# c-zhou/oatk

Measured on AMD Instinct MI355X. Metric: HiFi Gbases/s through syncasm (syncmer+syncerr) at k=1001 s=31, higher is better.
Workload: dtype u64

## Files before the change

oatk_amd/csrc/scan_syncmer_fast.hpp:

```cpp
#pragma once
#include <type_traits>
#include "common.hpp"
#include "scan_syncmer.hpp"
#include "scan_hpc.hpp"

namespace oatk {

constexpr int SYF_C = 8;
constexpr int SYF_T = SYN_NT * SYF_C;
constexpr int SYF_BLK = 64;
constexpr int SYF_LIST = 128;

static inline int syncmer_fast_ring(int K, int S)
{
    const int w = K - S;
    if (w / SYF_C - 1 < SYF_BLK || w / SYF_C - 1 >= 2 * SYF_BLK) return 0;
    if (K + SYF_T + SYF_C + 64 <= 4096) return 4096;
    return 0;
}

#define OATK_DPP_ROW_SHL(n) (0x100 + (n))
#define OATK_DPP_ROW_SHR(n) (0x110 + (n))
#define OATK_DPP_ROW_BCAST15 0x142
#define OATK_DPP_ROW_BCAST31 0x143

template <int CTRL, int ROW_MASK = 0xf>
__device__ __forceinline__ uint32_t dpp_u32(uint32_t old, uint32_t src)
{
    return (uint32_t) __builtin_amdgcn_update_dpp((int) old, (int) src, CTRL, ROW_MASK, 0xf, false);
}

__device__ __forceinline__ uint32_t wave_prefix_min_u32(uint32_t v)
{
    uint32_t p = v, t;
    t = dpp_u32<OATK_DPP_ROW_SHR(1)>(0xFFFFFFFFu, p); p = t < p? t : p;
    t = dpp_u32<OATK_DPP_ROW_SHR(2)>(0xFFFFFFFFu, p); p = t < p? t : p;
    t = dpp_u32<OATK_DPP_ROW_SHR(4)>(0xFFFFFFFFu, p); p = t < p? t : p;
    t = dpp_u32<OATK_DPP_ROW_SHR(8)>(0xFFFFFFFFu, p); p = t < p? t : p;
    t = dpp_u32<OATK_DPP_ROW_BCAST15, 0xa>(0xFFFFFFFFu, p); p = t < p? t : p;
    t = dpp_u32<OATK_DPP_ROW_BCAST31, 0xc>(0xFFFFFFFFu, p); p = t < p? t : p;
    return p;
}
__device__ __forceinline__ uint32_t wave_suffix_min_mirrored_u32(uint32_t v, uint32_t lane)
{
    return wave_prefix_min_u32((uint32_t) __builtin_amdgcn_ds_bpermute((int) ((63u - lane) << 2), (int) v));
}

#define OATK_SYF_PADW(R) ((R) / 8)
#ifndef OATK_SYF_EXP
#define OATK_SYF_EXP 0
#endif
#ifndef OATK_SYF_WAVES
#define OATK_SYF_WAVES 6
#endif
template <int R, bool S31, int NT, int SH>
__global__ __launch_bounds__(NT, OATK_SYF_WAVES) void syncmer_fast_kernel(SynArgs a)
{
    constexpr int C = SYF_C, T = NT * SYF_C, NCH = R / C, NWAVE = NT / OATK_WAVE;
    static_assert((R & (R - 1)) == 0, "power-of-two ring: index arithmetic is one AND (a 3200-slot ring raised occupancy from 3 to 4\n"
                  "workgroups per CU but its modulo arithmetic cost more issue slots than the occupancy returned)");

    __shared__ uint32_t m_top[R + OATK_SYF_PADW(R)];
    __shared__ uint64_t c_min[NCH];
    __shared__ uint32_t s_tie[2];
    __shared__ uint32_t pre32[NCH], suf32[NCH];
    __shared__ uint32_t w_cnt[2][NWAVE];
    __shared__ uint32_t sl_e[SYF_LIST];
    __shared__ uint32_t s_gb;

    const uint32_t r = blockIdx.x, tid = threadIdx.x, lane = tid & 63, wid = tid >> 6;
    if (a.n_nn[r] != 0) return;

    const int K = a.K, S = S31? 31 : a.S, w = K - S;
    const uint32_t hl = a.hoco_l[r];
    if (hl < (uint32_t) K) { if (tid == 0) a.n_scm[r] = 0; return; }
    const uint64_t sid = a.sid0 + r;
    const uint64_t mask = (1ULL << (2 * S)) - 1;
    const uint32_t *ghs = (const uint32_t *) (a.hoco_s + (a.off[r] >> 2));
    const int D = w / C - 1;

    auto rpos = [](int32_t i) -> uint32_t { return (uint32_t) i & (uint32_t) (R - 1); };
    auto mi = [&](int32_t i) -> uint32_t { const uint32_t p = rpos(i); return p + ((p >> 5) << 2); };
    auto rch = [](int32_t c) -> uint32_t { return (uint32_t) c & (uint32_t) (NCH - 1); };
    for (uint32_t i = tid; i < R + OATK_SYF_PADW(R); i += NT) m_top[i] = 0xFFFFFFFFu;
    for (uint32_t i = tid; i < NCH; i += NT) pre32[i] = suf32[i] = 0xFFFFFFFFu, c_min[i] = UINT64_MAX;
    if (tid < 2) s_tie[tid] = 0;
    __syncthreads();

    struct __attribute__((packed, aligned(4))) Words3 { uint32_t a, b, c; };
    const uint32_t bsel = (tid & 1u)? 0x06070001u : 0x04050607u;
    const uint32_t last_w = (hl - 1u) >> 4;
    uint32_t rw0, rw1, rw2;
    {
        const int32_t wi0 = ((int32_t) (tid * C) - 32) >> 4;
        rw0 = ghs[wi0 < 0? 0 : wi0], rw1 = ghs[wi0 + 1 < 0? 0 : wi0 + 1], rw2 = ghs[wi0 + 2];
    }

    uint32_t ord0 = 0, par = 0;
    uint32_t sl_n = 0;
    const uint32_t lcap = hl < (1u << 30)? (uint32_t) a.list_cap : 0u;
    const int HW = (w & (C - 1)) + C;

    auto get64g = [&](int32_t t) -> uint64_t {
        const uint32_t wi = (uint32_t) t >> 4, sh = ((uint32_t) t & 15u) * 2u;
        const uint64_t hi = (uint64_t) __builtin_bswap32(ghs[wi]) << 32 | __builtin_bswap32(ghs[wi + 1]);
        const uint32_t w2 = __builtin_bswap32(ghs[wi + 2]);
        return sh? (hi << sh) | ((uint64_t) w2 >> (32u - sh)) : hi;
    };
    auto hash_at = [&](int32_t q) -> uint64_t {
        if (q + 1 < S || (uint32_t) q >= hl) return UINT64_MAX;
        const uint64_t X = get64g(q - S + 1) & (~0ULL << (64 - 2 * S));
        const uint64_t fw = X >> (64 - 2 * S), rv = revcomp32(X) & mask;
        return S31? hash64_s31(fw < rv? fw : rv) : (fw != rv? hash64(fw < rv? fw : rv, mask) : UINT64_MAX);
    };
    auto write_record = [&](int32_t E, uint32_t kind, uint32_t loc, uint32_t ordn) __attribute__((always_inline)) {
        const int32_t e = kind == 2u? E - w : E, j = E - K + 1;
        const uint64_t X = get64g(e - S + 1) & (~0ULL << (64 - 2 * S));
        const uint64_t fw = X >> (64 - 2 * S), rv = revcomp32(X) & mask;
        uint64_t code = fw < rv? fw << 1 : rv << 1 | 1ULL;
        const uint32_t rev = (uint32_t) (code & 1ULL);
        if (kind == 1u) code ^= 1ULL;
        if (loc < a.region_cap) {
            const size_t slot = (size_t) (blockIdx.x & (OATK_REC_SHARDS - 1)) * a.region_cap + loc;
            a.rec_lo[slot] = sid << 32 | (uint64_t) ordn << 1 | rev;
            a.rec_smer[slot] = code;
            a.rec_mpos[slot] = (uint32_t) j << 1 | rev;
        }
    };
    auto emit_list = [&]() __attribute__((always_inline)) {
        if (sl_n) {
            if (tid == 0) s_gb = atomicAdd(&a.shard_cnt[blockIdx.x & (OATK_REC_SHARDS - 1)], sl_n);
            __syncthreads();
            const uint32_t gb = s_gb;
            for (uint32_t i = tid; i < sl_n; i += NT) write_record((int32_t) (sl_e[i] & 0x3FFFFFFFu), sl_e[i] >> 30, gb + i, ord0 + i);
            __syncthreads();
        }
        ord0 += sl_n, sl_n = 0;
    };

    uint32_t pend_kinds = 0, pend_rank = 0, pend_wtot = 0, pend_par = 0, pend_any = 0;
    int32_t pend_i0 = 0;
    auto flush = [&]() __attribute__((always_inline)) {
        if (!pend_any) return;
        uint32_t before = 0, tot = 0;
#pragma unroll
        for (int ww = 0; ww < NWAVE; ++ww) { const uint32_t c = w_cnt[pend_par][ww]; tot += c; before += ww < (int) wid? c : 0u; }
        pend_any = 0;
        if (tot == 0) return;
        if (sl_n + tot > lcap) emit_list();
        const bool direct = tot > lcap;
        if (direct) {
            if (tid == 0) s_gb = atomicAdd(&a.shard_cnt[blockIdx.x & (OATK_REC_SHARDS - 1)], tot);
            __syncthreads();
            uint32_t rank = before + pend_rank, kk = pend_kinds;
            while (kk) {
                const int o = __builtin_ctz(kk) >> 1;
                const uint32_t kind = (pend_kinds >> (2 * o)) & 3u;
                kk &= ~(3u << (2 * o));
                write_record(pend_i0 + o, kind, s_gb + rank, ord0 + rank);
                ++rank;
            }
            __syncthreads();
        } else if (pend_wtot) {
            uint32_t idx = sl_n + before + pend_rank, kk = pend_kinds;
            while (kk) {
                const int o = __builtin_ctz(kk) >> 1;
                sl_e[idx] = (uint32_t) (pend_i0 + o) | ((pend_kinds >> (2 * o)) & 3u) << 30;
                kk &= ~(3u << (2 * o));
                ++idx;
            }
        }
        ord0 += direct? tot : 0u;
        sl_n += direct? 0u : tot;
    };

    static_assert(2 * T == R, "the address toggling below needs tile = half the ring");
    struct RangeAddr { uint32_t lo, hi, mid; bool whole; };
    auto range_addr = [&](int32_t lo, int32_t hi) -> RangeAddr {
        return RangeAddr{rch(lo) * 4u, rch(hi) * 4u, rch(((lo >> 6) + 1) * 64 + 63) * 4u, (hi >> 6) - (lo >> 6) == 2};
    };
    const int32_t ch_0 = (int32_t) tid, ca0_0 = ((int32_t) (tid * C) - w) >> 3;
    RangeAddr rB = range_addr(ch_0 - D, ch_0 - 1), rF0 = range_addr(ca0_0 + 1, ca0_0 + D), rF1 = range_addr(ca0_0 + 2, ca0_0 + 1 + D);
    uint32_t o_cs = rch(ch_0) * 4u;
    uint32_t m_own = mi((int32_t) (tid * C)), m_fa = mi(ca0_0 * C), m_fb = mi((ca0_0 + 1) * C);
    const uint32_t m_own_sum = m_own + mi((int32_t) (tid * C) + T), m_fa_sum = m_fa + mi(ca0_0 * C + T), m_fb_sum = m_fb + mi((ca0_0 + 1) * C + T);
    auto next_tile_addr = [&]() __attribute__((always_inline)) {
        constexpr uint32_t FLIP = (uint32_t) (NCH / 2) * 4u;
        o_cs ^= FLIP;
        rB.lo ^= FLIP, rB.hi ^= FLIP, rB.mid ^= FLIP, rF0.lo ^= FLIP, rF0.hi ^= FLIP, rF0.mid ^= FLIP, rF1.lo ^= FLIP, rF1.hi ^= FLIP, rF1.mid ^= FLIP;
        m_own = m_own_sum - m_own, m_fa = m_fa_sum - m_fa, m_fb = m_fb_sum - m_fb;
    };
    auto ld32 = [](const uint32_t *base, uint32_t byte_off) -> uint32_t { return *(const uint32_t *) ((const char *) base + byte_off); };

    bool rep_mode = false, rep_next = false;
    int32_t rep_start = 0x7FFFFFFF;
    uint32_t quiet = 0, tpar = 0;
    const int32_t wave_first = __builtin_amdgcn_readfirstlane((int) (wid * OATK_WAVE * C));
    uint32_t I0 = 0;
    for (; I0 + (uint32_t) wave_first < hl; I0 += T, next_tile_addr(), tpar ^= 1u) {
        if (rep_next != rep_mode) { rep_mode = rep_next; rep_start = rep_mode? (int32_t) (I0 / C) : 0x7FFFFFFF; }
        const int32_t i0 = (int32_t) (I0 + tid * C);
        const int32_t wb = (int32_t) I0 + wave_first;
        const int32_t ch = i0 / C;
        uint32_t y[C];
        uint32_t cmin_keep;
        {
            const uint32_t a_hi = __builtin_amdgcn_perm(rw0, rw1, bsel), a_lo = __builtin_amdgcn_perm(rw1, rw2, bsel);
            const uint32_t vbh = __builtin_amdgcn_perm(rw2, 0u, bsel);
            const uint64_t vb = (uint64_t) vbh << 32;
            {
                const uint32_t wn = ((I0 + T + tid * C) - 32u) >> 4;
                const Words3 nx = *(const Words3 *) (ghs + (wn < last_w? wn : last_w));
                rw0 = nx.a, rw1 = nx.b, rw2 = nx.c;
            }
            uint64_t cm = UINT64_MAX;
            uint32_t cmin = 0xFFFFFFFFu;
            const bool inside = wb + 1 >= S && (uint32_t) (wb + OATK_WAVE * C) <= hl;
            if (S31 || inside) {
                if (S31) {
                    auto rc16 = [](uint32_t x) -> uint32_t {
                        const uint32_t r = __builtin_bitreverse32(x);
                        return ~(((r >> 1) & 0x55555555u) | ((r & 0x55555555u) << 1));
                    };
                    const uint32_t r0 = rc16(a_hi), r1 = rc16(a_lo), r2 = rc16(vbh);
                    auto hash_chunk = [&](auto keep, auto ends) __attribute__((always_inline)) {
#pragma unroll
                        for (int b = 0; b < C; ++b) {
                            uint64_t fw = (uint64_t) __builtin_amdgcn_alignbit(a_hi, a_lo, 28 - 2 * b) << 32 | __builtin_amdgcn_alignbit(a_lo, vbh, 28 - 2 * b);
                            uint64_t rv = (uint64_t) __builtin_amdgcn_alignbit(r2, r1, 2 + 2 * b) << 32 | __builtin_amdgcn_alignbit(r1, r0, 2 + 2 * b);
                            asm("" : "+v"(fw), "+v"(rv));
                            const uint64_t cn = fw < rv? fw : rv;
                            uint64_t mv4 = hash64_s31_left(cn);
                            y[b] = (uint32_t) (mv4 >> 34);
                            if (decltype(ends)::value) {
                                const bool ok = i0 + b + 1 >= S && (uint32_t) (i0 + b) < hl;
                                y[b] = ok? y[b] : 0xFFFFFFFFu;
                                if (decltype(keep)::value) mv4 = ok? mv4 : UINT64_MAX;
                            }
                            cmin = y[b] < cmin? y[b] : cmin;
                            if (decltype(keep)::value) cm = mv4 < cm? mv4 : cm;
                        }
                        if (decltype(keep)::value) cm = decltype(ends)::value && cm == UINT64_MAX? cm : cm >> 2;
                    };
                    if (inside) {
                        if (__builtin_amdgcn_readfirstlane((int) rep_mode)) hash_chunk(std::true_type(), std::false_type()); else hash_chunk(std::false_type(), std::false_type());
                    } else {
                        if (__builtin_amdgcn_readfirstlane((int) rep_mode)) hash_chunk(std::true_type(), std::true_type()); else hash_chunk(std::false_type(), std::true_type());
                    }
                } else {
                    const uint64_t X = ((uint64_t) a_hi << 32 | a_lo) << (2 * (32 - S));
                    uint64_t fw = X >> (64 - 2 * S), rv = revcomp32(X) & mask;
#pragma unroll
                    for (int b = 0; b < C; ++b) {
                        const uint64_t c = (vbh >> (30 - 2 * b)) & 3u;
                        fw = (fw << 2 | c) & mask;
                        rv = rv >> 2 | (3ULL ^ c) << (2 * S - 2);
                        const uint64_t mv = fw != rv? hash64(fw < rv? fw : rv, mask) : UINT64_MAX;
                        y[b] = (uint32_t) (mv >> 32);
                        cmin = y[b] < cmin? y[b] : cmin;
                        cm = mv < cm? mv : cm;
                    }
                }
            } else {
                const uint64_t X = ((uint64_t) a_hi << 32 | a_lo) << (2 * (32 - S));
                uint64_t fw = X >> (64 - 2 * S), rv = revcomp32(X) & mask;
#pragma unroll
                for (int b = 0; b < C; ++b) {
                    const int32_t i = i0 + b;
                    const uint64_t c = (vb >> (62 - 2 * b)) & 3ULL;
                    fw = (fw << 2 | c) & mask;
                    rv = rv >> 2 | (3ULL ^ c) << (2 * S - 2);
                    uint64_t mv = UINT64_MAX;
                    if (i + 1 >= S && (uint32_t) i < hl && fw != rv) mv = S31? hash64_s31(fw < rv? fw : rv) : hash64(fw < rv? fw : rv, mask);
                    y[b] = (uint32_t) (mv >> 32);
                    cmin = y[b] < cmin? y[b] : cmin;
                    if (rep_mode) cm = mv < cm? mv : cm;
                }
            }
            cmin_keep = cmin;
            uint32_t pre, suf;
#ifdef OATK_SCAN_SHFL
            pre = suf = cmin;
            for (int d = 1; d < OATK_WAVE; d <<= 1) {
                uint32_t up = __shfl_up(pre, d), dn = __shfl_down(suf, d);
                if ((int) lane >= d) pre = up < pre? up : pre;
                if ((int) lane + d < OATK_WAVE) suf = dn < suf? dn : suf;
            }
#else
            pre = wave_prefix_min_u32(cmin);
            suf = wave_suffix_min_mirrored_u32(cmin, lane);
#endif
            __syncthreads();
            static_assert(C == 8, "two 16-byte stores per lane");
            *(uint4 *) (m_top + m_own) = make_uint4(y[0], y[1], y[2], y[3]);
            *(uint4 *) (m_top + m_own + 4) = make_uint4(y[4], y[5], y[6], y[7]);
            if (rep_mode) *(uint64_t *) ((char *) c_min + 2u * o_cs) = cm;
            {
                const uint32_t seen = s_tie[tpar ^ 1u];
                quiet = seen? 0u : quiet + 1u;
                rep_next = seen != 0u || (rep_mode && quiet < 2u);
            }
            *(uint32_t *) ((char *) pre32 + o_cs) = pre;
#ifdef OATK_SCAN_SHFL
            *(uint32_t *) ((char *) suf32 + o_cs) = suf;
#else
            *(uint32_t *) ((char *) suf32 + (o_cs ^ 252u)) = suf;
#endif
        }
        __syncthreads();
        if (tid == 0) s_tie[tpar ^ 1u] = 0;
        flush();

        static_assert(SH >= 0 && SH < C, "the window's alignment against the chunks is a template argument");
        constexpr int RR = (C - SH) & (C - 1);
        uint32_t backF_keep = 0, fwd0_keep = 0, fwd1_keep = 0;
        uint32_t kinds = 0;
        uint32_t tiemask = 0;
        if (!(wb + OATK_WAVE * C < K)) {
            auto range_min = [&](const RangeAddr &ra) -> uint32_t {
                const uint32_t a0 = ld32(suf32, ra.lo), a1 = ld32(pre32, ra.hi);
                const uint32_t mid = ld32(pre32, ra.mid);
                const uint32_t a2 = ra.whole? mid : 0xFFFFFFFFu;
                const uint32_t v = a0 < a1? a0 : a1;
                return a2 < v? a2 : v;
            };
            const uint32_t backF = range_min(rB);
            const uint32_t fwd0 = range_min(rF0);
            const uint32_t fwd1 = range_min(rF1);
            backF_keep = backF, fwd0_keep = fwd0, fwd1_keep = fwd1;
            constexpr int BD = RR? RR : C;
            uint32_t W[2 * C];
            {
                const uint4 a0 = *(const uint4 *) (m_top + m_fa), a1 = *(const uint4 *) (m_top + m_fa + 4);
                const uint4 b0 = *(const uint4 *) (m_top + m_fb), b1 = *(const uint4 *) (m_top + m_fb + 4);
                const uint32_t all[2 * C] = {a0.x, a0.y, a0.z, a0.w, a1.x, a1.y, a1.z, a1.w, b0.x, b0.y, b0.z, b0.w, b1.x, b1.y, b1.z, b1.w};
#pragma unroll
                for (int j = 0; j < 2 * C - SH; ++j) W[j] = all[SH + j];
            }
            uint32_t cprev = 0xFFFFFFFFu;
            if (RR > 0) {
                const uint32_t nb = dpp_u32<0x138>(0xFFFFFFFFu, cmin_keep);
                const uint32_t lb = ld32(suf32, (o_cs - 4u) & (uint32_t) (NCH * 4 - 1));
                cprev = lane == 0? lb : nb;
            }
            const bool edge = !(wb + 1 >= K && (uint32_t) (wb + OATK_WAVE * C) <= hl);
            auto decide = [&](auto at_edge) __attribute__((always_inline)) {
#pragma unroll
                for (int o = 0; o < C; ++o) {
                    const uint32_t yhi = y[o], fhi = W[o];
                    const uint32_t fb = o + SH < C? fwd0 : fwd1;
                    const uint32_t fy = fb < yhi? fb : yhi;
                    const bool c1 = yhi <= backF, c2 = fhi <= fy;
                    uint64_t cand = __ballot(c1) | __ballot(c2);
                    bool fits = true;
                    if (decltype(at_edge)::value) {
                        fits = (uint32_t) (i0 + o) < hl && i0 + o + 1 >= K;
                        cand &= __ballot(fits);
                    }
#if OATK_SYF_EXP == 1
                    if (!a.want_n) cand = 0;
#endif
                    if (cand) {
                        const bool c = (c1 | c2) && fits;
                        uint32_t pmin = 0xFFFFFFFFu;
#pragma unroll
                        for (int j = 0; j < o; ++j) pmin = y[j] < pmin? y[j] : pmin;
                        const int cend = o < BD? BD - 1 : BD + C - 1;
                        uint32_t rest = 0xFFFFFFFFu;
#pragma unroll
                        for (int j = o + 1; j <= cend; ++j) rest = W[j] < rest? W[j] : rest;
                        uint32_t head = fhi < rest? fhi : rest;
                        if (o < RR) {
#pragma unroll
                            for (int j = RR; j < RR + C; ++j) head = W[j] < head? W[j] : head;
                        }
                        const uint32_t hb = head < backF? head : backF, bh = hb < pmin? hb : pmin;
                        const bool cl = yhi < bh, tie_c = yhi == bh;
                        const uint32_t tailp = o < RR? (cprev < pmin? cprev : pmin) : pmin;
                        const uint32_t rf = rest < fb? rest : fb, rh = rf < tailp? rf : tailp;
                        const bool le = fhi <= rh && fhi <= yhi, op = fhi < rh && fhi < yhi;
                        const bool tie = tie_c || (le && !op);
                        const uint32_t k = tie? 0u : (cl && op? 0u : (cl? 1u : (op? 2u : 0u)));
                        if (c) kinds |= k << (2 * o), tiemask |= (tie? 1u : 0u) << o;
                    }
                }
            };
            if (edge) decide(std::true_type()); else decide(std::false_type());
        }
        if (__ballot(tiemask != 0)) {
            constexpr int sh = SH;
            {
                if (lane == 0) s_tie[tpar] = 1u;
                const int32_t ca0_l = (i0 - w) >> 3;
                const int32_t c_lo = __builtin_amdgcn_readlane(ca0_l, 0) + 1, c_hi_all = __builtin_amdgcn_readlane(ca0_l, 63) + 1 + D;
                const int32_t c_hi = rep_mode && rep_start - 1 < c_hi_all? rep_start - 1 : c_hi_all;
                for (int32_t cc = c_lo + (int32_t) lane; cc <= c_hi; cc += 64) {
                    uint64_t u = UINT64_MAX;
                    for (int b = 0; b < C; ++b) { const uint64_t h = hash_at(cc * C + b); u = h < u? h : u; }
                    c_min[rch(cc)] = u;
                }
                __builtin_amdgcn_fence(__ATOMIC_RELEASE, "workgroup");
                __builtin_amdgcn_wave_barrier();
                __builtin_amdgcn_fence(__ATOMIC_ACQUIRE, "workgroup");
            }
            auto full = [&](int32_t q, uint32_t ref) -> uint64_t {
                const uint32_t t = m_top[mi(q)];
                return t == ref? hash_at(q) : (uint64_t) t << 32;
            };
            uint64_t r0 = UINT64_MAX, r1 = UINT64_MAX;
            if (tiemask) {
                const int32_t ca0 = (i0 - w) >> 3;
                uint64_t mid = UINT64_MAX;
                for (int32_t cc = ca0 + 2; cc <= ca0 + D; ++cc) { const uint64_t u = c_min[rch(cc)]; mid = u < mid? u : mid; }
                const uint64_t e0 = c_min[rch(ca0 + 1)], e1 = c_min[rch(ca0 + 1 + D)];
                r0 = e0 < mid? e0 : mid, r1 = e1 < mid? e1 : mid;
            }
            const uint64_t r_close = (w & (C - 1))? r1 : r0;
            uint32_t tm = tiemask;
            while (tm) {
                const int o = __builtin_ctz(tm);
                tm &= tm - 1;
                const int32_t E = i0 + o, lo = E - w;
                const uint32_t yhi = m_top[mi(E)], fhi = m_top[mi(lo)];
                const uint64_t yy = hash_at(E), f = hash_at(lo);
                const uint32_t fb = o + sh < C? fwd0_keep : fwd1_keep;
                bool cl = false, op = false;
                if (yhi <= backF_keep) {
                    uint64_t b = UINT64_MAX;
                    for (int t = 0; t < HW - o; ++t) { const uint64_t u = t? full(lo + t, yhi) : f; b = u < b? u : b; }
                    for (int t = 0; t < o; ++t) { const uint64_t u = full(i0 + t, yhi); b = u < b? u : b; }
                    if (yhi == backF_keep) b = r_close < b? r_close : b;
                    if (yy != UINT64_MAX && yy <= b) {
                        const uint64_t x = full(lo - 1, yhi);
                        cl = yy < b || x >= b || f == b;
                    }
                }
                if (fhi <= fb && fhi <= yhi) {
                    const int32_t ca = lo >> 3, tail0 = (ca + 1 + D) * C;
                    uint64_t b = UINT64_MAX;
                    for (int32_t q = lo + 1; q < (ca + 1) * C; ++q) { const uint64_t u = full(q, fhi); b = u < b? u : b; }
                    for (int32_t q = tail0; q < E; ++q) { const uint64_t u = full(q, fhi); b = u < b? u : b; }
                    if (fhi == fb) { const uint64_t u = ca == ((i0 - w) >> 3)? r0 : r1; b = u < b? u : b; }
                    op = f != UINT64_MAX && f <= b && f <= yy;
                }
                kinds |= (cl && op? 0u : (cl? 1u : (op? 2u : 0u))) << (2 * o);
            }
        }
#if OATK_SYF_EXP == 5
        kinds &= (uint32_t) -a.want_n;
#endif
        const uint32_t ns = (uint32_t) __builtin_popcount((kinds | kinds >> 1) & 0x5555u);
        const uint32_t incl = wave_incl_sum_dpp(ns, lane);
        const uint32_t wtot = (uint32_t) __builtin_amdgcn_readlane((int) incl, 63);
        if (lane == 0) w_cnt[par][wid] = wtot;
        pend_kinds = kinds, pend_rank = incl - ns, pend_i0 = i0, pend_wtot = wtot, pend_par = par, pend_any = 1u;
        par ^= 1u;
    }
    if (I0 < hl) {
        __syncthreads();
        __syncthreads();
        flush();
        if (lane == 0) w_cnt[par][wid] = 0;
        pend_kinds = 0, pend_rank = 0, pend_wtot = 0, pend_par = par, pend_any = 1u;
    }
    __syncthreads();
    flush();
    __syncthreads();
    emit_list();
    if (tid == 0) a.n_scm[r] = ord0;
}

}
```

Measured before the change: 406.6.

## Trim per-lane registers and instructions in syncmer fast scan loop

Drops the separate backward-range descriptor by reusing a forward range min, and recomputes the tie-path range mins on demand instead of carrying keep registers. Converts ring offsets to byte units, and uses bitop3 for the reverse-complement plus direct compare-mask intrinsics in place of ballots. Makes the repeat-mode flag scalar through a branchless update, and stores a per-tile base instead of a per-lane i0 for the pending flush. The goal is lower VGPR pressure and fewer ALU and LDS-address instructions per tile. The backF substitution relies on the window geometry making the two ranges equivalent, so a mismatch there would be a correctness risk.

```diff
diff --git a/oatk_amd/csrc/scan_syncmer_fast.hpp b/oatk_amd/csrc/scan_syncmer_fast.hpp
--- a/oatk_amd/csrc/scan_syncmer_fast.hpp
+++ b/oatk_amd/csrc/scan_syncmer_fast.hpp
@@ -23,6 +23,7 @@
 #define OATK_DPP_ROW_SHR(n) (0x110 + (n))
 #define OATK_DPP_ROW_BCAST15 0x142
 #define OATK_DPP_ROW_BCAST31 0x143
+#define OATK_ICMP_ULE 37
 
 template <int CTRL, int ROW_MASK = 0xf>
 __device__ __forceinline__ uint32_t dpp_u32(uint32_t old, uint32_t src)
@@ -90,6 +91,7 @@
     struct __attribute__((packed, aligned(4))) Words3 { uint32_t a, b, c; };
     const uint32_t bsel = (tid & 1u)? 0x06070001u : 0x04050607u;
     const uint32_t last_w = (hl - 1u) >> 4;
+    const uint32_t lane_w4 = (uint32_t) ((((int32_t) (tid * C) - 32) >> 4) * 4);
     uint32_t rw0, rw1, rw2;
     {
         const int32_t wi0 = ((int32_t) (tid * C) - 32) >> 4;
@@ -139,7 +141,7 @@
     };
 
     uint32_t pend_kinds = 0, pend_rank = 0, pend_wtot = 0, pend_par = 0, pend_any = 0;
-    int32_t pend_i0 = 0;
+    uint32_t pend_I0 = 0;
     auto flush = [&]() __attribute__((always_inline)) {
         if (!pend_any) return;
         uint32_t before = 0, tot = 0;
@@ -153,6 +155,7 @@
             if (tid == 0) s_gb = atomicAdd(&a.shard_cnt[blockIdx.x & (OATK_REC_SHARDS - 1)], tot);
             __syncthreads();
             uint32_t rank = before + pend_rank, kk = pend_kinds;
+            const int32_t pend_i0 = (int32_t) (pend_I0 + tid * C);
             while (kk) {
                 const int o = __builtin_ctz(kk) >> 1;
                 const uint32_t kind = (pend_kinds >> (2 * o)) & 3u;
@@ -163,6 +166,7 @@
             __syncthreads();
         } else if (pend_wtot) {
             uint32_t idx = sl_n + before + pend_rank, kk = pend_kinds;
+            const int32_t pend_i0 = (int32_t) (pend_I0 + tid * C);
             while (kk) {
                 const int o = __builtin_ctz(kk) >> 1;
                 sl_e[idx] = (uint32_t) (pend_i0 + o) | ((pend_kinds >> (2 * o)) & 3u) << 30;
@@ -175,24 +179,25 @@
     };
 
     static_assert(2 * T == R, "the address toggling below needs tile = half the ring");
-    struct RangeAddr { uint32_t lo, hi, mid; bool whole; };
+    struct RangeAddr { uint32_t lo, hi, mid; };
     auto range_addr = [&](int32_t lo, int32_t hi) -> RangeAddr {
-        return RangeAddr{rch(lo) * 4u, rch(hi) * 4u, rch(((lo >> 6) + 1) * 64 + 63) * 4u, (hi >> 6) - (lo >> 6) == 2};
+        const bool whole = (hi >> 6) - (lo >> 6) == 2;
+        return RangeAddr{rch(lo) * 4u, rch(hi) * 4u, rch(whole? ((lo >> 6) + 1) * 64 + 63 : hi) * 4u};
     };
     const int32_t ch_0 = (int32_t) tid, ca0_0 = ((int32_t) (tid * C) - w) >> 3;
-    RangeAddr rB = range_addr(ch_0 - D, ch_0 - 1), rF0 = range_addr(ca0_0 + 1, ca0_0 + D), rF1 = range_addr(ca0_0 + 2, ca0_0 + 1 + D);
+    RangeAddr rF0 = range_addr(ca0_0 + 1, ca0_0 + D), rF1 = range_addr(ca0_0 + 2, ca0_0 + 1 + D);
     uint32_t o_cs = rch(ch_0) * 4u;
-    uint32_t m_own = mi((int32_t) (tid * C)), m_fa = mi(ca0_0 * C), m_fb = mi((ca0_0 + 1) * C);
-    const uint32_t m_own_sum = m_own + mi((int32_t) (tid * C) + T), m_fa_sum = m_fa + mi(ca0_0 * C + T), m_fb_sum = m_fb + mi((ca0_0 + 1) * C + T);
+    uint32_t m_own = mi((int32_t) (tid * C)) * 4u, m_fa = mi(ca0_0 * C) * 4u, m_fb = mi((ca0_0 + 1) * C) * 4u;
+    const uint32_t m_own_sum = m_own + mi((int32_t) (tid * C) + T) * 4u, m_fa_sum = m_fa + mi(ca0_0 * C + T) * 4u, m_fb_sum = m_fb + mi((ca0_0 + 1) * C + T) * 4u;
     auto next_tile_addr = [&]() __attribute__((always_inline)) {
         constexpr uint32_t FLIP = (uint32_t) (NCH / 2) * 4u;
         o_cs ^= FLIP;
-        rB.lo ^= FLIP, rB.hi ^= FLIP, rB.mid ^= FLIP, rF0.lo ^= FLIP, rF0.hi ^= FLIP, rF0.mid ^= FLIP, rF1.lo ^= FLIP, rF1.hi ^= FLIP, rF1.mid ^= FLIP;
+        rF0.lo ^= FLIP, rF0.hi ^= FLIP, rF0.mid ^= FLIP, rF1.lo ^= FLIP, rF1.hi ^= FLIP, rF1.mid ^= FLIP;
         m_own = m_own_sum - m_own, m_fa = m_fa_sum - m_fa, m_fb = m_fb_sum - m_fb;
     };
     auto ld32 = [](const uint32_t *base, uint32_t byte_off) -> uint32_t { return *(const uint32_t *) ((const char *) base + byte_off); };
 
-    bool rep_mode = false, rep_next = false;
+    uint32_t rep_mode = 0, rep_next = 0;
     int32_t rep_start = 0x7FFFFFFF;
     uint32_t quiet = 0, tpar = 0;
     const int32_t wave_first = __builtin_amdgcn_readfirstlane((int) (wid * OATK_WAVE * C));
@@ -209,8 +214,8 @@
             const uint32_t vbh = __builtin_amdgcn_perm(rw2, 0u, bsel);
             const uint64_t vb = (uint64_t) vbh << 32;
             {
-                const uint32_t wn = ((I0 + T + tid * C) - 32u) >> 4;
-                const Words3 nx = *(const Words3 *) (ghs + (wn < last_w? wn : last_w));
+                const uint32_t wn4 = (I0 + T) / 4u + lane_w4;
+                const Words3 nx = *(const Words3 *) ((const char *) ghs + (wn4 < last_w * 4u? wn4 : last_w * 4u));
                 rw0 = nx.a, rw1 = nx.b, rw2 = nx.c;
             }
             uint64_t cm = UINT64_MAX;
@@ -220,7 +225,7 @@
                 if (S31) {
                     auto rc16 = [](uint32_t x) -> uint32_t {
                         const uint32_t r = __builtin_bitreverse32(x);
-                        return ~(((r >> 1) & 0x55555555u) | ((r & 0x55555555u) << 1));
+                        return (uint32_t) __builtin_amdgcn_bitop3_b32((int) (r >> 1), (int) (r << 1), 0x55555555, 0x1b);
                     };
                     const uint32_t r0 = rc16(a_hi), r1 = rc16(a_lo), r2 = rc16(vbh);
                     auto hash_chunk = [&](auto keep, auto ends) __attribute__((always_inline)) {
@@ -243,9 +248,9 @@
                         if (decltype(keep)::value) cm = decltype(ends)::value && cm == UINT64_MAX? cm : cm >> 2;
                     };
                     if (inside) {
-                        if (__builtin_amdgcn_readfirstlane((int) rep_mode)) hash_chunk(std::true_type(), std::false_type()); else hash_chunk(std::false_type(), std::false_type());
+                        if (rep_mode) hash_chunk(std::true_type(), std::false_type()); else hash_chunk(std::false_type(), std::false_type());
                     } else {
-                        if (__builtin_amdgcn_readfirstlane((int) rep_mode)) hash_chunk(std::true_type(), std::true_type()); else hash_chunk(std::false_type(), std::true_type());
+                        if (rep_mode) hash_chunk(std::true_type(), std::true_type()); else hash_chunk(std::false_type(), std::true_type());
                     }
                 } else {
                     const uint64_t X = ((uint64_t) a_hi << 32 | a_lo) << (2 * (32 - S));
@@ -292,13 +297,12 @@
 #endif
             __syncthreads();
             static_assert(C == 8, "two 16-byte stores per lane");
-            *(uint4 *) (m_top + m_own) = make_uint4(y[0], y[1], y[2], y[3]);
-            *(uint4 *) (m_top + m_own + 4) = make_uint4(y[4], y[5], y[6], y[7]);
-            if (rep_mode) *(uint64_t *) ((char *) c_min + 2u * o_cs) = cm;
+            *(uint4 *) ((char *) m_top + m_own) = make_uint4(y[0], y[1], y[2], y[3]);
+            *(uint4 *) ((char *) m_top + m_own + 16) = make_uint4(y[4], y[5], y[6], y[7]);
             {
-                const uint32_t seen = s_tie[tpar ^ 1u];
-                quiet = seen? 0u : quiet + 1u;
-                rep_next = seen != 0u || (rep_mode && quiet < 2u);
+                const uint32_t seen = (uint32_t) __builtin_amdgcn_readfirstlane((int) s_tie[tpar ^ 1u]);
+                quiet = (quiet + 1u) & (seen - 1u);
+                rep_next = seen | (rep_mode & ((quiet - 2u) >> 31));
             }
             *(uint32_t *) ((char *) pre32 + o_cs) = pre;
 #ifdef OATK_SCAN_SHFL
@@ -306,6 +310,7 @@
 #else
             *(uint32_t *) ((char *) suf32 + (o_cs ^ 252u)) = suf;
 #endif
+            if (rep_mode) *(uint64_t *) ((char *) c_min + 2u * o_cs) = cm;
         }
         __syncthreads();
         if (tid == 0) s_tie[tpar ^ 1u] = 0;
@@ -313,35 +318,30 @@
 
         static_assert(SH >= 0 && SH < C, "the window's alignment against the chunks is a template argument");
         constexpr int RR = (C - SH) & (C - 1);
-        uint32_t backF_keep = 0, fwd0_keep = 0, fwd1_keep = 0;
         uint32_t kinds = 0;
         uint32_t tiemask = 0;
+        auto range_min = [&](const RangeAddr &ra) -> uint32_t {
+            const uint32_t a0 = ld32(suf32, ra.lo), a1 = ld32(pre32, ra.hi), a2 = ld32(pre32, ra.mid);
+            const uint32_t v = a0 < a1? a0 : a1;
+            return a2 < v? a2 : v;
+        };
         if (!(wb + OATK_WAVE * C < K)) {
-            auto range_min = [&](const RangeAddr &ra) -> uint32_t {
-                const uint32_t a0 = ld32(suf32, ra.lo), a1 = ld32(pre32, ra.hi);
-                const uint32_t mid = ld32(pre32, ra.mid);
-                const uint32_t a2 = ra.whole? mid : 0xFFFFFFFFu;
-                const uint32_t v = a0 < a1? a0 : a1;
-                return a2 < v? a2 : v;
-            };
-            const uint32_t backF = range_min(rB);
             const uint32_t fwd0 = range_min(rF0);
             const uint32_t fwd1 = range_min(rF1);
-            backF_keep = backF, fwd0_keep = fwd0, fwd1_keep = fwd1;
+            const uint32_t backF = RR? fwd1 : fwd0;
             constexpr int BD = RR? RR : C;
             uint32_t W[2 * C];
             {
-                const uint4 a0 = *(const uint4 *) (m_top + m_fa), a1 = *(const uint4 *) (m_top + m_fa + 4);
-                const uint4 b0 = *(const uint4 *) (m_top + m_fb), b1 = *(const uint4 *) (m_top + m_fb + 4);
+                const uint4 a0 = *(const uint4 *) ((const char *) m_top + m_fa), a1 = *(const uint4 *) ((const char *) m_top + m_fa + 16);
+                const uint4 b0 = *(const uint4 *) ((const char *) m_top + m_fb), b1 = *(const uint4 *) ((const char *) m_top + m_fb + 16);
                 const uint32_t all[2 * C] = {a0.x, a0.y, a0.z, a0.w, a1.x, a1.y, a1.z, a1.w, b0.x, b0.y, b0.z, b0.w, b1.x, b1.y, b1.z, b1.w};
 #pragma unroll
                 for (int j = 0; j < 2 * C - SH; ++j) W[j] = all[SH + j];
             }
             uint32_t cprev = 0xFFFFFFFFu;
             if (RR > 0) {
-                const uint32_t nb = dpp_u32<0x138>(0xFFFFFFFFu, cmin_keep);
                 const uint32_t lb = ld32(suf32, (o_cs - 4u) & (uint32_t) (NCH * 4 - 1));
-                cprev = lane == 0? lb : nb;
+                cprev = dpp_u32<0x138>(lb, cmin_keep);
             }
             const bool edge = !(wb + 1 >= K && (uint32_t) (wb + OATK_WAVE * C) <= hl);
             auto decide = [&](auto at_edge) __attribute__((always_inline)) {
@@ -350,8 +350,7 @@
                     const uint32_t yhi = y[o], fhi = W[o];
                     const uint32_t fb = o + SH < C? fwd0 : fwd1;
                     const uint32_t fy = fb < yhi? fb : yhi;
-                    const bool c1 = yhi <= backF, c2 = fhi <= fy;
-                    uint64_t cand = __ballot(c1) | __ballot(c2);
+                    uint64_t cand = __builtin_amdgcn_uicmp(yhi, backF, OATK_ICMP_ULE) | __builtin_amdgcn_uicmp(fhi, fy, OATK_ICMP_ULE);
                     bool fits = true;
                     if (decltype(at_edge)::value) {
                         fits = (uint32_t) (i0 + o) < hl && i0 + o + 1 >= K;
@@ -361,7 +360,7 @@
                     if (!a.want_n) cand = 0;
 #endif
                     if (cand) {
-                        const bool c = (c1 | c2) && fits;
+                        const bool c = (yhi <= backF || fhi <= fy) && fits;
                         uint32_t pmin = 0xFFFFFFFFu;
 #pragma unroll
                         for (int j = 0; j < o; ++j) pmin = y[j] < pmin? y[j] : pmin;
@@ -389,6 +388,8 @@
         }
         if (__ballot(tiemask != 0)) {
             constexpr int sh = SH;
+            const int32_t i0 = (int32_t) ((uint32_t) __builtin_amdgcn_readfirstlane((int) I0) + tid * C);
+            const uint32_t fwd0_keep = range_min(rF0), fwd1_keep = range_min(rF1), backF_keep = RR? fwd1_keep : fwd0_keep;
             {
                 if (lane == 0) s_tie[tpar] = 1u;
                 const int32_t ca0_l = (i0 - w) >> 3;
@@ -453,7 +454,7 @@
         const uint32_t incl = wave_incl_sum_dpp(ns, lane);
         const uint32_t wtot = (uint32_t) __builtin_amdgcn_readlane((int) incl, 63);
         if (lane == 0) w_cnt[par][wid] = wtot;
-        pend_kinds = kinds, pend_rank = incl - ns, pend_i0 = i0, pend_wtot = wtot, pend_par = par, pend_any = 1u;
+        pend_kinds = kinds, pend_rank = incl - ns, pend_I0 = I0, pend_wtot = wtot, pend_par = par, pend_any = 1u;
         par ^= 1u;
     }
     if (I0 < hl) {
```

Result: faster. 420.5 (median of 6 runs) (+3.4%).
